# refresh-bio/DSRC

Hardware: AMD Instinct MI355X
Metric: raw FASTQ MB/s compressed (bit-identical .dsrc) at -d3 -q2 (higher is better)
Workload: dtype u8/u16/u32 integer

## Files before the change

### dsrc_amd/csrc/dsrc_gpu.hip

```cpp
#include <hip/hip_runtime.h>

#include <algorithm>
#include <atomic>
#include <cstdarg>
#include <cstdio>
#include <cstdlib>
#include <cstring>
#include <chrono>
#include <condition_variable>
#include <deque>
#include <functional>
#include <dlfcn.h>
#include <mutex>
#ifndef DSRC_REPLAY_WHATIF
#define DSRC_REPLAY_WHATIF 0
#endif
#include <string>
#include <thread>
#include <vector>

#include "../../include/dsrc_gpu.h"
#include "dsrc_types.h"
#include "k_common.h"
#ifndef RCS_WIDE
// ... 656 lines not shown
			hb = std::min(hb, j.key_bits);
			if (j.key_bits > BK_MAX_LB) hb = std::max(hb, j.key_bits - BK_MAX_LB);
			j.bk_hb = hb; j.bk_lb = j.key_bits - hb;
			j.bk_mul = BK_HASH_MUL; j.bk_kmask = (u32)((1ull << j.key_bits) - 1ull);
			j.bk_limit = bk_limit; j.bk_big = bk_big;
			j.bk_narrow_bins = (u32)std::min<long>(BK_MAX_BINS, hook_int("DSRC_GPU_BUCKET_NARROW_BINS", BK_MAX_BINS));
		}
		bk_zero_words = cur;
		o_bk = A.alloc(((size_t)cur + 2 + 128) * 4 + 64);
		size_t cnt_words = 0;
		for (u32 i = 0; i < NJ; ++i)
			if (jobs[i].bk_on)
			{
				if (cnt_words >= (1ull << 32)) return fail(h, DSRCGPU_E_NOMEM, "batch too large for the bucket count table");
				jobs[i].bk_cnt = (u32)cnt_words;
				cnt_words += (((size_t)jobs[i].n + BK_BIN - 1) >> BK_TB) << jobs[i].bk_hb;
			}
		o_bcnt = A.alloc(cnt_words * 2 + 64);
	}
	for (u32 i = 0; i < NJ; ++i) chains[i].bk_on = use_bk ? jobs[i].bk_on : 0u;
	const size_t o_redo = A.alloc(((size_t)NJ + 2) * 4);
	const size_t o_jobs = A.alloc(sizeof(CtxJob) * std::max(1u, NJ)), o_chains = A.alloc(sizeof(RcChain) * std::max(1u, NJ));
	if (A.failed) return fail(h, DSRCGPU_E_NOMEM, "arena exhausted (phase 3b): batch needs > %zu bytes of HBM scratch", A.top);
	CtxJob* d_jobs = AP<CtxJob>(h, o_jobs); RcChain* d_chains = AP<RcChain>(h, o_chains);

	HIPCHK(hipMemcpyAsync(st.data(), d_state, sizeof(BlkState) * B, hipMemcpyDeviceToHost, s));
	HIPCHK(hipStreamSynchronize(s));
	mark("S3"); tr.stage("dsrc batch: tags, order models, range coder");
	std::vector<TagFieldRes> tres((size_t)B * DSRC_MAX_FIELDS);
	memset(tres.data(), 0, sizeof(TagFieldRes) * tres.size());
	size_t tz_lo = al(A.top, 256); A.top = tz_lo;
	for (u32 b = 0; b < B; ++b)
	{
		const BlkState& S = st[b]; BlkDesc& D = desc[b];
		size_t words = 0, hdr = 64;
		tplan[b].rbits_off = (u32)words; words += S.n_recs + 4;
		tplan[b].raw_hist_off = (u32)words; words += 128 + h_huff_ws_words(128) + h_huff_tree_cap(128) / 4 + 16;
		for (u32 fi = 0; fi < S.n_fields && !S.mixed; ++fi)
		{
			const TagField& f = S.fld[fi];
			TagFieldRes& R = tres[(size_t)b * DSRC_MAX_FIELDS + fi];
			hdr += 32 + f.len0 + f.len0 / 8;
			if (f.is_string)
			{
				R.hist_off = (u32)words; words += 129 * 256;
				R.ham_off = (u32)words; words += f.len0 + 4;
				R.code_off = (u32)words; words += 129 * 256;
				R.len_off = (u32)words; words += 129 * 256;
				R.tree_slot = 4 + h_huff_tree_cap(256);
				R.tree_off = (u32)(words * 4); words += ((size_t)129 * R.tree_slot + 3) / 4;
				R.ws_slot = h_huff_ws_words(256); R.ws_off = (u32)words; words += (size_t)129 * R.ws_slot;
				hdr += (size_t)129 * R.tree_slot;
			}
			else if (f.is_numeric && !f.is_constant && f.var_stat_encode)
			{
				R.hist_off = (u32)words; words += 512;
				R.code_off = (u32)words; words += 512;
				R.len_off = (u32)words; words += 512;
				R.tree_slot = 4 + h_huff_tree_cap(512);
				R.tree_off = (u32)(words * 4); words += (R.tree_slot + 3) / 4;
				R.ws_slot = h_huff_ws_words(512); R.ws_off = (u32)words; words += R.ws_slot;
				hdr += R.tree_slot;
			}
		}
		if (S.mixed) hdr += 64 + h_huff_tree_cap(128);
		tplan[b].scr = A.alloc(words * 4) / 4;
		const size_t cap_bytes = hdr + ((size_t)S.raw_tag * 9 + 7) / 8 + (size_t)S.n_recs * ((size_t)S.n_fields * 5 + 8) + 64;
		D.tag_cap = (u32)(al(cap_bytes, 16) / 4 + 4);
		D.tag_out = A.alloc((size_t)D.tag_cap * 4) / 4;
	}
	size_t tz_hi = al(A.top, 256); A.top = tz_hi;
	if (A.failed) return fail(h, DSRCGPU_E_NOMEM, "arena exhausted (tags): batch needs > %zu bytes of HBM scratch", A.top);
	HIPCHK(hipMemsetAsync(h->arena.base + tz_lo, 0, tz_hi - tz_lo, s));
	HIPCHK(hipMemcpyAsync(d_desc, desc.data(), sizeof(BlkDesc) * B, hipMemcpyHostToDevice, s));
	HIPCHK(hipMemcpyAsync(d_tplan, tplan.data(), sizeof(TagPlan) * B, hipMemcpyHostToDevice, s));
	HIPCHK(hipMemcpyAsync(d_tres, tres.data(), sizeof(TagFieldRes) * tres.size(), hipMemcpyHostToDevice, s));
	hipLaunchKernelGGL(k_tag_hist, dim3(B), dim3(WG), 0, s, d_in, d_desc, d_state, rp, wpool, wpool, d_tplan, d_tres); KCHK();
	hipLaunchKernelGGL(k_tag_trees, dim3((DSRC_MAX_FIELDS * DSRC_MAX_STRF + 63) / 64, B), dim3(64), 0, s, d_state, wpool, d_tplan, d_tres); KCHK();
	hipLaunchKernelGGL(k_tag_emit, dim3(B), dim3(WG), 0, s, d_in, d_desc, d_state, rp, wpool, spool, wpool, wpool, d_tplan, d_tres); KCHK();
	hipLaunchKernelGGL(k_tag_raw, dim3(B), dim3(WG), 0, s, d_in, d_desc, d_state, rp, wpool, wpool, d_tplan); KCHK();

	if (zero_hi > zero_lo) HIPCHK(hipMemsetAsync(h->arena.base + zero_lo, 0, zero_hi - zero_lo, s));
	HIPCHK(hipMemcpyAsync(d_desc, desc.data(), sizeof(BlkDesc) * B, hipMemcpyHostToDevice, s));
	HIPCHK(hipMemcpyAsync(d_qplan, qplan.data(), sizeof(QuaPlan) * B, hipMemcpyHostToDevice, s));
	HIPCHK(hipMemcpyAsync(d_dplan, dplan.data(), sizeof(QuaPlan) * B, hipMemcpyHostToDevice, s));
	if (NJ)
	{
		HIPCHK(hipMemcpyAsync(d_jobs, jobs.data(), sizeof(CtxJob) * NJ, hipMemcpyHostToDevice, s));
		HIPCHK(hipMemcpyAsync(d_chains, chains.data(), sizeof(RcChain) * NJ, hipMemcpyHostToDevice, s));
	}

	u32 maxq = 1, maxd = 1, max_len = 1, max_qn = 1;
	for (u32 b = 0; b < B; ++b) { maxq = std::max(maxq, st[b].q_total); maxd = std::max(maxd, st[b].d_total); max_len = std::max(max_len, st[b].max_len); max_qn = std::max(max_qn, st[b].q_count); }

	if (qo == 0)
	{
		hipLaunchKernelGGL(k_qpos_hist, dim3(B), dim3(WG), 0, s, d_desc, d_state, rp, d_q, wpool, d_qplan); KCHK();
		hipLaunchKernelGGL(k_qpos_trees, dim3((max_len + 63) / 64, B), dim3(64), 0, s, d_state, wpool, d_qplan); KCHK();
		hipLaunchKernelGGL(k_qpos_emit, dim3(B), dim3(WG), 0, s, d_desc, d_state, rp, d_q, wpool, wpool, d_qplan); KCHK();
		hipLaunchKernelGGL(k_qrle_runs, dim3(B), dim3(WG), 0, s, d_desc, d_state, d_q, wpool, d_qplan); KCHK();
		hipLaunchKernelGGL(k_qrle_hist, dim3(B), dim3(WG), 0, s, d_desc, d_state, d_q, wpool, d_qplan); KCHK();
		hipLaunchKernelGGL(k_qrle_trees, dim3((2 * max_qn + 63) / 64, B), dim3(64), 0, s, d_state, wpool, d_qplan); KCHK();
		hipLaunchKernelGGL(k_qrle_emit, dim3(B), dim3(WG), 0, s, d_desc, d_state, d_q, wpool, wpool, d_qplan); KCHK();
	}
	if (dna_order == 0)
	{
		const u32 gx = std::max(1u, std::min(64u, (maxd / 4 + WG - 1) / WG));
		hipLaunchKernelGGL(k_dna_b2, dim3(gx, B), dim3(WG), 0, s, d_desc, d_state, d_d, wpool); KCHK();
		hipLaunchKernelGGL(k_dna_huff, dim3(B), dim3(WG), 0, s, d_desc, d_state, d_d, wpool, wpool, d_dplan); KCHK();
	}
	hipLaunchKernelGGL(k_dna_none, dim3((B + 63) / 64), dim3(64), 0, s, d_desc, d_state, wpool, B); KCHK();
	h->rc_launches = 0;
	std::function<int(const BkGroup&)> launch_fallback;
	u32* d_bk = use_bk ? AP<u32>(h, o_bk) : nullptr;
	u32* d_redo = AP<u32>(h, o_redo);
	const bool rc_one_lane = hook_env("DSRC_GPU_RC_ONE_LANE") != nullptr;
	if (NJ)
	{
		const u32 nq = (u32)qjobs.size(), nd = (u32)djobs.size();
		const bool sort_atomic = h->sort_atomic;
		hipLaunchKernelGGL(k_rc_headers, dim3((NJ + 63) / 64), dim3(64), 0, s, d_jobs, NJ, d_state, wpool); KCHK();
		HIPCHK(hipMemsetAsync(d_redo, 0, ((size_t)NJ + 2) * 4, s));
		u16* d_bcnt = use_bk ? AP<u16>(h, o_bcnt) : nullptr;
		if (use_bk) HIPCHK(hipMemsetAsync(d_bk, 0, bk_zero_words * 4, s));
		const u32 max_parts = 2048u;
		launch_fallback = [&, sort_atomic, max_parts](const BkGroup& g) -> int
		{
			const u32 cnt = g.hi - g.lo;
			const u32* fb = d_bk + g.fb;
			if (sort_atomic) hipLaunchKernelGGL((k_sort<0, true>), dim3(std::min(cnt, 16u)), dim3(SORT_WG), 0, s, d_jobs, lpool, d_d, d_q, d_qp, d_state, fb);
			else hipLaunchKernelGGL((k_sort<0, false>), dim3(std::min(cnt, 16u)), dim3(SORT_WG), 0, s, d_jobs, lpool, d_d, d_q, d_qp, d_state, fb);
			u32 mxn = 1; for (u32 i = g.lo; i < g.hi; ++i) mxn = std::max(mxn, jobs[i].n);
			const u32 parts = std::max(1u, std::min(max_parts, mxn / 1024u));
			const dim3 rgrid(parts * std::min(cnt, 4u));
#define BK_REPLAY(NN) { hipLaunchKernelGGL(k_replay_seams<NN>, rgrid, dim3(REPLAY_WG), 0, s, d_jobs, const_cast<u64*>(lpool), parts, cnt, fb); \
					hipLaunchKernelGGL((k_replay<NN, 0>), rgrid, dim3(REPLAY_WG), 0, s, d_jobs, lpool, AP<RcPack>(h, 0), parts, cnt, fb); }
			switch (jobs[g.lo].n_alpha)
			{
			case 4: BK_REPLAY(4) break; case 8: BK_REPLAY(8) break; case 16: BK_REPLAY(16) break;
			case 32: BK_REPLAY(32) break; case 64: BK_REPLAY(64) break; default: BK_REPLAY(128) break;
			}
#undef BK_REPLAY
			KCHK();
			return 0;
		};
		for (size_t sl = 0; sl + 1 < slice_lo.size(); ++sl)
		{
			const u32 s_lo = slice_lo[sl], s_hi = slice_lo[sl + 1];
			stage_mark(0);
			if (use_bk)
			{
				u32 slice_bins = 0;
				for (u32 i = s_lo; i < s_hi; ++i) if (jobs[i].bk_on) slice_bins = std::max(slice_bins, (jobs[i].n + BK_BIN - 1) >> BK_TB);
				hipLaunchKernelGGL(k_part, dim3(std::max(1u, slice_bins), s_hi - s_lo), dim3(PART_WG), 0, s, d_jobs + s_lo, lpool, d_d, d_q, d_qp, d_state, d_bk, d_bcnt);
				KCHK();
				stage_mark(0); stage_mark(1);
				if (slice_bins) { hipLaunchKernelGGL(k_binoff, dim3(slice_bins, s_hi - s_lo), dim3(256), 0, s, d_jobs + s_lo, d_bcnt, d_bk); KCHK(); }
				for (const BkGroup& g : bk_groups[sl])
				{
					u32 hb = 0; bool any = false;
					for (u32 i = g.lo; i < g.hi; ++i) if (jobs[i].bk_on) { any = true; hb = std::max(hb, jobs[i].bk_hb); }
					if (!any) continue;
					u32 lbm = 0; for (u32 i = g.lo; i < g.hi; ++i) if (jobs[i].bk_on) lbm = std::max(lbm, jobs[i].bk_lb);
#define BK_LAUNCH(NN, MB, RB) hipLaunchKernelGGL((k_model<NN, MB, RB>), dim3(((1u << hb) + MD_WAVES_FOR(RB) - 1) / MD_WAVES_FOR(RB), g.hi - g.lo), dim3(64 * MD_WAVES_FOR(RB)), 0, s, d_jobs + g.lo, lpool, AP<RcPack>(h, 0), d_bk, d_bcnt, (RcPack*)(d_bk + ((bk_zero_words + 1) & ~(size_t)1)))
#define BK_FINISH(NN) { if ((1u << lbm) * 4 * MdRow<NN>::STRIDE <= 4096) BK_LAUNCH(NN, 0, 4096); \
						else if ((1u << lbm) * 4 * MdRow<NN>::STRIDE <= MD_ROW_BYTES) BK_LAUNCH(NN, 0, MD_ROW_BYTES); \
						else if (lbm <= 10) BK_LAUNCH(NN, 10, MD_ROW_BYTES); \
						else BK_LAUNCH(NN, BK_MAX_LB, MD_ROW_BYTES); }
					switch (jobs[g.lo].n_alpha)
					{
					case 4: BK_FINISH(4) break; case 8: BK_FINISH(8) break; case 16: BK_FINISH(16) break;
					case 32: BK_FINISH(32) break; case 64: BK_FINISH(64) break; default: BK_FINISH(128) break;
					}
#undef BK_LAUNCH
#undef BK_FINISH
					KCHK();
				}
				if (bk_binned && slice_bins) { hipLaunchKernelGGL(k_place, dim3(slice_bins, s_hi - s_lo), dim3(PLACE_WG), 0, s, d_jobs + s_lo, lpool, AP<RcPack>(h, 0), d_bk); KCHK(); }
				for (const BkGroup& g : bk_groups[sl])
				{
					bool known = false;
					for (u32 i = g.lo; i < g.hi; ++i) known = known || !jobs[i].bk_on;
					if (known) { const int rc = launch_fallback(g); if (rc) return rc; }
				}
				stage_mark(1);
				continue;
			}
#ifdef DSRC_SORT_PROBE
			{
				static int shots = 0;
				if (sl == 0 && shots < 2)
				{
					++shots;
					hipEvent_t e0, e1; hipEventCreate(&e0); hipEventCreate(&e1);
#define PROBE_RUN(M) { hipEventRecord(e0, s); if (sort_atomic) hipLaunchKernelGGL((k_sort<M, true>), dim3(s_hi - s_lo), dim3(SORT_WG), 0, s, d_jobs + s_lo, lpool, d_d, d_q, d_qp, d_state, nullptr); else hipLaunchKernelGGL((k_sort<M, false>), dim3(s_hi - s_lo), dim3(SORT_WG), 0, s, d_jobs + s_lo, lpool, d_d, d_q, d_qp, d_state, nullptr); \
					hipEventRecord(e1, s); hipEventSynchronize(e1); float ms = 0; hipEventElapsedTime(&ms, e0, e1); fprintf(stderr, "[probe] k_sort<%u> %u streams: %.2f ms\n", (unsigned)M, s_hi - s_lo, ms); }
					PROBE_RUN(0) PROBE_RUN(0) PROBE_RUN(128) PROBE_RUN(129) PROBE_RUN(130) PROBE_RUN(132) PROBE_RUN(134) PROBE_RUN(136) PROBE_RUN(144) PROBE_RUN(160) PROBE_RUN(192) PROBE_RUN(255)
					hipEventDestroy(e0); hipEventDestroy(e1);
				}
			}
#endif
			if (sort_atomic) hipLaunchKernelGGL((k_sort<0, true>), dim3(s_hi - s_lo), dim3(SORT_WG), 0, s, d_jobs + s_lo, lpool, d_d, d_q, d_qp, d_state, nullptr);
			else hipLaunchKernelGGL((k_sort<0, false>), dim3(s_hi - s_lo), dim3(SORT_WG), 0, s, d_jobs + s_lo, lpool, d_d, d_q, d_qp, d_state, nullptr);
			KCHK();
			stage_mark(0); stage_mark(1);
			for (u32 lo = s_lo; lo < s_hi;)
			{
				u32 hi = lo;
				while (hi < s_hi && jobs[hi].n_alpha == jobs[lo].n_alpha) ++hi;
				const u32 cnt = hi - lo;
				u32 mxn = 1; for (u32 i = lo; i < hi; ++i) mxn = std::max(mxn, jobs[i].n);
				const u32 parts = std::max(1u, std::min(max_parts, mxn / 1024u));
				const dim3 rgrid(parts * cnt);
#ifdef DSRC_SORT_PROBE
				{
					static int shots = 0;
					if ((jobs[lo].n_alpha == 32 || jobs[lo].n_alpha == 4) && lo == s_lo && shots < 4 && (sl == 0 || sl + 2 == slice_lo.size()))
					{
						++shots;
						hipEvent_t e0, e1; hipEventCreate(&e0); hipEventCreate(&e1);
#define RPROBE_RUN(NN, M) { hipEventRecord(e0, s); hipLaunchKernelGGL((k_replay<NN, M>), rgrid, dim3(REPLAY_WG), 0, s, d_jobs + lo, lpool, AP<RcPack>(h, 0), parts, cnt, nullptr); \
						hipEventRecord(e1, s); hipEventSynchronize(e1); float ms = 0; hipEventElapsedTime(&ms, e0, e1); fprintf(stderr, "[probe] k_replay<%d,%d> %u streams x %u parts: %.2f ms\n", NN, M, cnt, parts, ms); }
						hipLaunchKernelGGL(k_replay_seams<32>, rgrid, dim3(REPLAY_WG), 0, s, d_jobs + lo, const_cast<u64*>(lpool), parts, cnt, nullptr);
						if (jobs[lo].n_alpha == 32) { RPROBE_RUN(32, 0) RPROBE_RUN(32, 0) RPROBE_RUN(32, 1) RPROBE_RUN(32, 2) RPROBE_RUN(32, 8) RPROBE_RUN(32, 16) }
						else { RPROBE_RUN(4, 0) RPROBE_RUN(4, 0) RPROBE_RUN(4, 1) RPROBE_RUN(4, 2) RPROBE_RUN(4, 8) RPROBE_RUN(4, 16) }
						hipEventDestroy(e0); hipEventDestroy(e1);
					}
				}
#endif
				switch (jobs[lo].n_alpha)
				{
				case 4:   hipLaunchKernelGGL(k_replay_seams<4>, rgrid, dim3(REPLAY_WG), 0, s, d_jobs + lo, const_cast<u64*>(lpool), parts, cnt, nullptr); hipLaunchKernelGGL((k_replay<4, DSRC_REPLAY_WHATIF>), rgrid, dim3(REPLAY_WG), 0, s, d_jobs + lo, lpool, AP<RcPack>(h, 0), parts, cnt, nullptr); break;
				case 8:   hipLaunchKernelGGL(k_replay_seams<8>, rgrid, dim3(REPLAY_WG), 0, s, d_jobs + lo, const_cast<u64*>(lpool), parts, cnt, nullptr); hipLaunchKernelGGL((k_replay<8, DSRC_REPLAY_WHATIF>), rgrid, dim3(REPLAY_WG), 0, s, d_jobs + lo, lpool, AP<RcPack>(h, 0), parts, cnt, nullptr); break;
				case 16:  hipLaunchKernelGGL(k_replay_seams<16>, rgrid, dim3(REPLAY_WG), 0, s, d_jobs + lo, const_cast<u64*>(lpool), parts, cnt, nullptr); hipLaunchKernelGGL((k_replay<16, DSRC_REPLAY_WHATIF>), rgrid, dim3(REPLAY_WG), 0, s, d_jobs + lo, lpool, AP<RcPack>(h, 0), parts, cnt, nullptr); break;
				case 32:  hipLaunchKernelGGL(k_replay_seams<32>, rgrid, dim3(REPLAY_WG), 0, s, d_jobs + lo, const_cast<u64*>(lpool), parts, cnt, nullptr); hipLaunchKernelGGL((k_replay<32, DSRC_REPLAY_WHATIF>), rgrid, dim3(REPLAY_WG), 0, s, d_jobs + lo, lpool, AP<RcPack>(h, 0), parts, cnt, nullptr); break;
				case 64:  hipLaunchKernelGGL(k_replay_seams<64>, rgrid, dim3(REPLAY_WG), 0, s, d_jobs + lo, const_cast<u64*>(lpool), parts, cnt, nullptr); hipLaunchKernelGGL((k_replay<64, DSRC_REPLAY_WHATIF>), rgrid, dim3(REPLAY_WG), 0, s, d_jobs + lo, lpool, AP<RcPack>(h, 0), parts, cnt, nullptr); break;
				default:  hipLaunchKernelGGL(k_replay_seams<128>, rgrid, dim3(REPLAY_WG), 0, s, d_jobs + lo, const_cast<u64*>(lpool), parts, cnt, nullptr); hipLaunchKernelGGL((k_replay<128, DSRC_REPLAY_WHATIF>), rgrid, dim3(REPLAY_WG), 0, s, d_jobs + lo, lpool, AP<RcPack>(h, 0), parts, cnt, nullptr); break;
				}
				KCHK();
				lo = hi;
			}
			stage_mark(1);
		}
		HIPCHK(hipEventRecord(h->ev[4], s));
		HIPCHK(hipStreamWaitEvent(h->rc_stream, h->ev[4], 0));
		HIPCHK(hipEventRecord(h->ev[2], h->rc_stream));
		if (rc_one_lane) hipLaunchKernelGGL(k_rc, dim3((NJ + RC_LANES - 1) / RC_LANES), dim3(64 * RC_WG_WAVES), 0, h->rc_stream, d_chains, NJ, (const u32*)nullptr, AP<RcPack>(h, 0), wpool, d_state);
		else if (NJ > (u32)hook_int("DSRC_GPU_RC_WIDE_FROM", 640)) hipLaunchKernelGGL(k_rcs<RCS_WIDE>, dim3((NJ + RCS_WIDE - 1) / RCS_WIDE), dim3(64 * RCS_WG_WAVES), 0, h->rc_stream, d_chains, NJ, AP<RcPack>(h, 0), wpool, d_state, (const u32*)d_bk, d_redo);
		else hipLaunchKernelGGL(k_rcs<16>, dim3((NJ + 15) / 16), dim3(64 * RCS_WG_WAVES), 0, h->rc_stream, d_chains, NJ, AP<RcPack>(h, 0), wpool, d_state, (const u32*)d_bk, d_redo);
		KCHK();
		HIPCHK(hipEventRecord(h->ev[3], h->rc_stream));
		HIPCHK(hipEventSynchronize(h->ev[3]));
		h->rc_launches = 1;
	}

	hipLaunchKernelGGL(k_meta_plan, dim3((B + 63) / 64), dim3(64), 0, s, d_state, prm); KCHK();

	HIPCHK(hipMemcpyAsync(st.data(), d_state, sizeof(BlkState) * B, hipMemcpyDeviceToHost, s));
	std::vector<u32> bk_flags, redo;
	if (NJ)
	{
		redo.resize((size_t)NJ + 1); HIPCHK(hipMemcpyAsync(redo.data(), d_redo, ((size_t)NJ + 1) * 4, hipMemcpyDeviceToHost, s));
		if (use_bk) { bk_flags.resize(NJ); HIPCHK(hipMemcpyAsync(bk_flags.data(), d_bk, (size_t)NJ * 4, hipMemcpyDeviceToHost, s)); }
	}
	HIPCHK(hipStreamSynchronize(s));
	if (NJ && !rc_one_lane)
	{
		std::vector<u32> list(redo.begin() + 1, redo.begin() + 1 + std::min<u32>(redo[0], NJ));
		u32 why[4] = {0, 0, 0, 0};
		for (u32& x : list) { ++why[(x >> 28) & 3u]; x &= 0x0FFFFFFFu; }
		bool handed = false;
		for (u32 i = 0; i < NJ && use_bk; ++i) if (bk_flags[i] && jobs[i].bk_on) { list.push_back(i); handed = true; }
		if (!list.empty())
		{
			mark("redo"); tr.stage("dsrc batch: range coder, redo list");
			if (handed)
				for (size_t sl = 0; sl + 1 < slice_lo.size(); ++sl)
					for (const BkGroup& g : bk_groups[sl])
					{
						bool any = false;
						for (u32 i = g.lo; i < g.hi; ++i) any = any || (bk_flags[i] && jobs[i].bk_on);
						if (any) { const int rc = launch_fallback(g); if (rc) return rc; }
					}
			std::sort(list.begin(), list.end()); list.erase(std::unique(list.begin(), list.end()), list.end());
			std::vector<u32> up(list.size() + 1); up[0] = (u32)list.size(); std::copy(list.begin(), list.end(), up.begin() + 1);
			HIPCHK(hipMemcpyAsync(d_redo, up.data(), up.size() * 4, hipMemcpyHostToDevice, s));
			hipLaunchKernelGGL(k_rc, dim3(((u32)list.size() + RC_LANES - 1) / RC_LANES), dim3(64 * RC_WG_WAVES), 0, s, d_chains, NJ, (const u32*)d_redo, AP<RcPack>(h, 0), wpool, d_state); KCHK();
			HIPCHK(hipMemcpyAsync(st.data(), d_state, sizeof(BlkState) * B, hipMemcpyDeviceToHost, s));
			HIPCHK(hipStreamSynchronize(s));
			h->rc_redone += (u32)list.size();
			if (getenv("DSRC_GPU_DEBUG")) fprintf(stderr, "[dsrc_gpu] range coder: %zu of %u streams coded again by k_rc (%u carry clamps: fix row taken %u, recovery refused %u, forced %u; the others handed back by the bucketed front end)\n", list.size(), NJ, std::min<u32>(redo[0], NJ), why[1], why[2], why[3]);
		}
	}
	mark("S4"); tr.stage("dsrc batch: assemble");
	if (!bk_flags.empty() && getenv("DSRC_GPU_DEBUG"))
	{
		u32 on = 0, back = 0;
		for (u32 i = 0; i < NJ; ++i) { on += jobs[i].bk_on; back += bk_flags[i] && jobs[i].bk_on; }
		fprintf(stderr, "[dsrc_gpu] bucketed path: %u of %u streams tried, %u handed back to k_sort / k_replay\n", on, NJ, back);
	}
	u64 total = 0;
	for (u32 b = 0; b < B; ++b)
	{
		const BlkState& S = st[b];
		if ((S.err & DSRC_ERR_OUT_OVERFLOW) && !h->rc_caps_worst && NJ)
		{
			h->rc_caps_worst = true; A.failed = true;
			return fail(h, DSRCGPU_E_NOMEM, "chunk %u: a range-coded stream outgrew its staging estimate; the batch is run again with worst-case staging", b);
// ... 1375 lines not shown
```

### dsrc_amd/csrc/k_bucket.h

```cpp
#pragma once
#include <type_traits>
#include "k_rc.h"

#define BK_MAX_HB 10
#define BK_MAX_LB 11
#define BK_LIMIT 524288
#define BK_BIG 16384
#ifndef BK_TB
#define BK_TB 13
#endif
#define BK_BIN (1u << BK_TB)
static_assert(BK_TB == RC6_TB, "a time bin is the unit of k_rc's record layout (rc6_chunk_off)");
#ifndef BK_MAX_BINS
#define BK_MAX_BINS 512
#endif
#define BK_MAX_BINS_WIDE 65536
#define BK_HASH_MUL 0x9E3779B1u


__device__ __forceinline__ u64 bk_rekey(const CtxJob& j, u64 el)
{
	const u32 key = ((u32)(el >> ELEM_CTX_SHIFT) * j.bk_mul) & j.bk_kmask;
	return (el & ((1ull << ELEM_CTX_SHIFT) - 1ull)) | ((u64)key << ELEM_CTX_SHIFT);
}

__device__ __forceinline__ void bk_fallback(const CtxJob& j, u32* bk)
{
	if (atomicExch(&bk[j.jid], 1u) != 0u) return;
	const u32 k = atomicAdd(&bk[j.bk_fb], 1u);
	bk[j.bk_fb + 1 + k] = j.jid;
}

__device__ __forceinline__ bool bk_fast8(const CtxJob& j) { return j.is_dna ? (j.alpha_bits == 2 && j.order <= 9) : j.order <= 4; }

struct BkWin { u64 a, b, c; };
__device__ __forceinline__ BkWin bk_load8(const CtxJob& j, const u8* s, u32 t0)
{
	BkWin w;
	if (j.is_dna) { w.a = *(const u64_unaligned*)(s + t0 - 9); w.b = *(const u64_unaligned*)(s + t0 - 1); w.c = *(const u64_unaligned*)(s + t0); }
	else { w.a = *(const u64_unaligned*)(s + t0 - 8); w.b = 0; w.c = *(const u64_unaligned*)(s + t0); }
	return w;
}

__device__ __forceinline__ void bk_elems8_dna(const CtxJob& j, const BkWin& w, u32 t0, u64* el, bool* bad)
{
	const u64 wa = w.a, wb = w.b, wc = w.c;
	if ((wa | wc) & 0xFCFCFCFCFCFCFCFCull) *bad = true;
	const u32 P = (pack2x8(__builtin_bswap64(wa)) << 16) | pack2x8(__builtin_bswap64(wb));
	const u32 cmask = (u32)((1ull << (2 * j.order)) - 1ull);
#pragma unroll
	for (u32 i = 0; i < 8; ++i)
	{
		const u32 ctx = (P >> (14 - 2 * i)) & cmask;
		const u32 key = (ctx * j.bk_mul) & j.bk_kmask;
		el[i] = ((u64)key << ELEM_CTX_SHIFT) | ((u64)((u32)(wc >> (8 * i)) & 3u) << ELEM_SYM_SHIFT) | (t0 + i);
	}
}

__device__ __forceinline__ void bk_elems8_qua(const CtxJob& j, const BkWin& w, const u8* qp, const u8* rank, u32 t0, u64* el)
{
	const u32 ab = j.alpha_bits, order = j.order, half = order / 2;
	const u64 w0 = w.a, w1 = w.c;
	u32 r[16];
#pragma unroll
	for (u32 m = 0; m < 8; ++m) { r[m] = rank[(u32)(w0 >> (8 * m)) & 0xFFu]; r[8 + m] = rank[(u32)(w1 >> (8 * m)) & 0xFFu]; }
	u32 pos = j.qlen ? t0 - exact_div(t0, j.qm_lo, j.qm_hi) * j.qlen : 0u;
#pragma unroll
	for (u32 i = 0; i < 8; ++i)
	{
		u32 h = 0;
#pragma unroll
		for (u32 k = 4; k >= 1; --k)
			if (k <= order)
			{
				const u32 slot = k - 1;
				const u32 x = (slot < half || order == 1) ? r[7 + i - slot] : ((r[7 + i - slot] + r[6 + i - slot]) >> 1);
				h = (h << ab) | x;
			}
		const u32 pctx = (j.qlen ? exact_div(pos * 128u, j.qm_lo, j.qm_hi) : (u32)qp[t0 + i]) >> j.rescale_shift;
		const u32 key = ((((h << ab) | pctx)) * j.bk_mul) & j.bk_kmask;
		el[i] = ((u64)key << ELEM_CTX_SHIFT) | ((u64)(r[8 + i] & ((1u << ab) - 1u)) << ELEM_SYM_SHIFT) | (t0 + i);
		pos = pos + 1 == j.qlen ? 0u : pos + 1;
	}
}

#ifndef PART_ITEMS
#define PART_ITEMS 16
#endif
#define PART_WG (BK_BIN / PART_ITEMS)
#ifndef PART_PASSES
#define PART_PASSES 1
#endif
#define PART_WAVES (PART_WG / 64)
#define BK_EL_SYM_SHIFT BK_TB
#define BK_EL_KEY_SHIFT (BK_TB + 7)
static_assert(BK_EL_KEY_SHIFT + BK_MAX_LB <= 32, "low key bits, symbol and time inside the tile in 32 bits");
__device__ __forceinline__ u32 bk_keysym(u64 e) { return ((u32)(e >> (ELEM_SYM_SHIFT + 1)) & ~0x7Fu) | ((u32)(e >> ELEM_SYM_SHIFT) & 0x7Fu); }
static_assert(ELEM_CTX_SHIFT == ELEM_SYM_SHIFT + 8, "bk_keysym");

__global__ void __launch_bounds__(PART_WG) k_part(const CtxJob* jobs, u64* pool, const u8* d_stream, const u8* q_stream, const u8* qp_stream, BlkState* st, u32* bk, u16* bcnt)
{
	__shared__ u16 s_cnt[PART_WAVES][SORT_MAX_BINS];
	__shared__ u32 s_tile[BK_BIN / PART_PASSES];
	__shared__ u32 s_ws[PART_WAVES];
	__shared__ u8 s_rank[256];
	constexpr u32 tile_elems = PART_WG * PART_ITEMS;
	const CtxJob j = jobs[blockIdx.y];
	if (!j.bk_on) { if (blockIdx.x == 0 && threadIdx.x == 0) bk_fallback(j, bk); return; }
	const u32 tile = blockIdx.x * tile_elems;
	if (tile >= j.n) return;
	const u32 n = j.n, bins = 1u << j.bk_hb, lb = j.bk_lb;
	const u32 wv = wave_id(), lane = lane_id();
	const u8* sym_src = (j.is_dna ? d_stream : q_stream) + j.src_off;
	const u8* qp = qp_stream + j.src_off;

	for (u32 i = threadIdx.x; i < 256; i += blockDim.x) s_rank[i] = (!j.is_dna && j.translate) ? st[j.blk].q_sym[i] : (u8)i;
	for (u32 i = threadIdx.x; i < PART_WAVES * SORT_MAX_BINS / 2; i += blockDim.x) ((u32*)&s_cnt[0][0])[i] = 0;
	__syncthreads();

	u32 ks[PART_ITEMS], rk[PART_ITEMS];
	const u32 wbase = tile + wv * 64 * PART_ITEMS;
	bool bad = false;
	if (bk_fast8(j) && tile > 0 && tile + tile_elems + 8 <= n)
	{
		static_assert(PART_ITEMS % 8 == 0, "eight consecutive symbols per lane and round");
		static_assert(PART_WAVES * 512 <= BK_BIN / PART_PASSES, "a strip of 512 elements per wave");
		u32* strip = s_tile + wv * 512;
		BkWin w = bk_load8(j, sym_src, wbase + 8 * lane);
#pragma unroll
		for (u32 h = 0; h < PART_ITEMS / 8; ++h)
		{
			u64 e8[8];
			const u32 t0 = wbase + 512 * h + 8 * lane;
			const BkWin wc = w;
			if (h + 1 < PART_ITEMS / 8) w = bk_load8(j, sym_src, t0 + 512);
			if (j.is_dna) bk_elems8_dna(j, wc, t0, e8, &bad); else bk_elems8_qua(j, wc, qp, s_rank, t0, e8);
			if (h) wave_fence();
#pragma unroll
			for (u32 k = 0; k < 8; ++k) strip[8 * lane + k] = bk_keysym(e8[k]);
			wave_fence();
#pragma unroll
			for (u32 k = 0; k < 8; ++k) ks[8 * h + k] = strip[64 * k + lane];
		}
	}
	else
	{
#pragma unroll
		for (u32 k = 0; k < PART_ITEMS; ++k)
		{
			const u32 i = wbase + k * 64 + lane;
			ks[k] = 0;
			if (i < n)
			{
				const u64 e = bk_rekey(j, j.is_dna ? ctx_elem_dna(j, sym_src, i, &bad) : ctx_elem_qua(j, sym_src, qp, s_rank, i));
				ks[k] = bk_keysym(e);
			}
		}
	}
	if (bad) atomicOr(&st[j.blk].err, (u32)DSRC_ERR_REF_UB);
	const u32 shift = 7 + lb;
#pragma unroll
	for (u32 k = 0; k < PART_ITEMS; ++k)
	{
		const u32 i = wbase + k * 64 + lane;
		const u32 d = ks[k] >> shift;
		const u32 sh = (d & 1u) * 16u;
		u32 old = 0;
		if (i < n) old = atomicAdd(&((u32*)s_cnt[wv])[d >> 1], 1u << sh);
		rk[k] = (old >> sh) & 0xFFFFu;
#ifdef DSRC_EMU_BUILD
		(void)__ballot(true);
#endif
	}
	__syncthreads();
	for (u32 d0 = 0, carry = 0; d0 < bins; d0 += PART_WG)
	{
		const u32 dd = d0 + threadIdx.x;
		u32 c[PART_WAVES], tot = 0;
#pragma unroll
		for (u32 w = 0; w < PART_WAVES; ++w) { c[w] = dd < bins ? s_cnt[w][dd] : 0u; tot += c[w]; }
		const u32 inc = wave_incl_scan_dpp(tot);
		if (lane == 63) s_ws[wv] = inc;
		__syncthreads();
		u32 run = carry + inc - tot;
		const u32 nws = (bins - d0 + 63) / 64 < PART_WAVES ? (bins - d0 + 63) / 64 : PART_WAVES;
		for (u32 i = 0; i < nws; ++i) { const u32 x = s_ws[i]; run += i < wv ? x : 0u; carry += x; }
		if (dd < bins)
		{
			bcnt[(u64)j.bk_cnt + (u64)blockIdx.x * bins + dd] = (u16)tot;
#pragma unroll
			for (u32 w = 0; w < PART_WAVES; ++w) { s_cnt[w][dd] = (u16)run; run += c[w]; }
		}
		if (d0 + PART_WG < bins) __syncthreads();
	}
	__syncthreads();
	const u32 lbmask = (1u << lb) - 1u;
	u32* dst = (u32*)(pool + j.elems) + tile;
	const u32 tile_n = n - tile < tile_elems ? n - tile : tile_elems;
	constexpr u32 PIECE = BK_BIN / PART_PASSES;
#pragma unroll
	for (u32 k = 0; k < PART_ITEMS; ++k) rk[k] += (u32)s_cnt[wv][ks[k] >> shift];
#pragma unroll
	for (u32 p = 0; p < PART_PASSES; ++p)
	{
#pragma unroll
		for (u32 k = 0; k < PART_ITEMS; ++k)
		{
			const u32 i = wbase + k * 64 + lane;
			const u32 at = rk[k] - p * PIECE;
			if (i < n && at < PIECE)
				s_tile[at] = (((ks[k] >> 7) & lbmask) << BK_EL_KEY_SHIFT) | ((ks[k] & 0x7Fu) << BK_EL_SYM_SHIFT) | (i & (BK_BIN - 1u));
		}
		__syncthreads();
		if (tile_n == tile_elems)
		{
#pragma unroll
			for (u32 k = 0; k < PIECE / 2 / PART_WG; ++k) ((u64*)(dst + p * PIECE))[k * PART_WG + threadIdx.x] = ((const u64*)s_tile)[k * PART_WG + threadIdx.x];
		}
		else for (u32 q = threadIdx.x; q < PIECE && p * PIECE + q < tile_n; q += PART_WG) dst[p * PIECE + q] = s_tile[q];
		if (p + 1 < PART_PASSES) __syncthreads();
	}
}

#define MD_WAVES_FOR(ROW_BYTES) ((ROW_BYTES) <= 4096 ? 4 : 2)
#define MD_ROW_BYTES 8192
#define MD_NONE 0xFFFFFFFFu

template <int N> struct MdRow
{
	static constexpr int B = N <= 4 ? 2 : N <= 8 ? 3 : N <= 16 ? 4 : N <= 32 ? 5 : N <= 64 ? 6 : 7;
	static constexpr int L4 = B / 2;
	static constexpr bool R2 = (B & 1) != 0;
	static constexpr u32 W64 = ((1u << (2 * L4)) - 1u) / 3u;
	static constexpr u32 STRIDE = 2 * W64 + (R2 ? N / 2 : 0);
};

template <int N> __device__ __forceinline__ u32 md_init_word(u32 x)
{
	typedef MdRow<N> G;
	if (x >= 2 * G::W64) return 0x00010001u;
	const u32 w = x >> 1;
	const u32 l = w >= 5 ? 2u : w >= 1 ? 1u : 0u;
	const u32 v = (u32)N >> (2 * (l + 1));
	return v | (v << 16);
}

template <int N> __device__ __forceinline__ u32 md_total(const u32* row)
{
	const u64 v = *(const unsigned long long*)row;
	return ((u32)v & 0xFFFFu) + ((u32)v >> 16) + ((u32)(v >> 32) & 0xFFFFu) + (u32)(v >> 48);
}

template <int N> __device__ __forceinline__ void md_rescale(u32* row)
{
	typedef MdRow<N> G;
	unsigned long long* r64 = (unsigned long long*)row;
	if (G::R2)
		for (u32 x = 0; x < (u32)N / 2; ++x)
		{
			const u32 v = row[2 * G::W64 + x];
			u32 a = v & 0xFFFFu, b = v >> 16;
			a -= a >> 1; b -= b >> 1;
			row[2 * G::W64 + x] = a | (b << 16);
		}
	for (int l = G::L4 - 1; l >= 0; --l)
	{
		const u32 base = ((1u << (2 * l)) - 1u) / 3u, nw = 1u << (2 * l);
		for (u32 w = 0; w < nw; ++w)
		{
			u64 v = 0;
			if (!G::R2 && l == G::L4 - 1)
			{
				const u64 o = r64[base + w];
#pragma unroll
				for (u32 q = 0; q < 4; ++q) { u32 x = (u32)(o >> (16 * q)) & 0xFFFFu; x -= x >> 1; v |= (u64)x << (16 * q); }
			}
			else
			{
#pragma unroll
				for (u32 q = 0; q < 4; ++q)
				{
					const u32 c = 4 * w + q;
					u32 sum;
					if (l == G::L4 - 1) { const u32 p = row[2 * G::W64 + c]; sum = (p & 0xFFFFu) + (p >> 16); }
					else { const u64 o = r64[((1u << (2 * (l + 1))) - 1u) / 3u + c]; sum = ((u32)o & 0xFFFFu) + ((u32)o >> 16) + ((u32)(o >> 32) & 0xFFFFu) + (u32)(o >> 48); }
					v |= (u64)sum << (16 * q);
				}
			}
			r64[base + w] = v;
		}
	}
}

template <int N> __device__ __forceinline__ u64 md_code(u32* row, u32 sym)
{
	typedef MdRow<N> G;
	unsigned long long* r64 = (unsigned long long*)row;
	u32 cum = 0, tot = 0, f = 0;
#pragma unroll
	for (int l = 0; l < G::L4; ++l)
	{
		const u32 q = (sym >> (G::B - 2 * l - 2)) & 3u;
		const u32 wi = ((1u << (2 * l)) - 1u) / 3u + (l ? sym >> (G::B - 2 * l) : 0u);
		const u64 old = atomicAdd(&r64[wi], 2ull << (16 * q));
		const u64 below = old & ((1ull << (16 * q)) - 1ull);
		cum += ((u32)below & 0xFFFFu) + ((u32)below >> 16) + ((u32)(below >> 32) & 0xFFFFu);
		if (l == 0) tot = ((u32)old & 0xFFFFu) + ((u32)old >> 16) + ((u32)(old >> 32) & 0xFFFFu) + (u32)(old >> 48);
		f = (u32)(old >> (16 * q)) & 0xFFFFu;
	}
	if (G::R2)
	{
		const u32 old = atomicAdd(&row[2 * G::W64 + (sym >> 1)], (sym & 1u) ? (2u << 16) : 2u);
		cum += (sym & 1u) ? (old & 0xFFFFu) : 0u;
		f = (sym & 1u) ? (old >> 16) : (old & 0xFFFFu);
	}
	return (u64)f | ((u64)cum << 16) | ((u64)tot << 32);
}

__global__ void __launch_bounds__(256) k_binoff(const CtxJob* jobs, u16* bcnt, const u32* bk)
{
	const CtxJob j = jobs[blockIdx.y];
	const u32 bin = blockIdx.x;
	if (!j.bk_on || bk[j.jid] || (bin << BK_TB) >= j.n) return;
	const u32 bins = 1u << j.bk_hb;
	u16* row = bcnt + j.bk_cnt + (u64)bin * bins;
	u32 c[4], mine = 0;
#pragma unroll
	for (u32 k = 0; k < 4; ++k)
	{
		const u32 b = 4 * threadIdx.x + k;
		c[k] = b < bins ? (u32)row[b] : 0u;
		mine += c[k];
	}
	u32 tot;
	u32 run = block_excl_scan(mine, &tot);
#pragma unroll
	for (u32 k = 0; k < 4; ++k)
	{
		const u32 b = 4 * threadIdx.x + k;
		if (b < bins) row[b] = (u16)run;
		run += c[k];
	}
}

template <bool SMALL> struct MdMapT { typedef u8 T; static constexpr u32 NONE = 0xFFu, CLAIM = 0x80u; };
template <> struct MdMapT<false> { typedef u16 T; static constexpr u32 NONE = 0xFFFFu, CLAIM = 0x8000u; };

#ifndef MD_AHEAD
#define MD_AHEAD 3
#endif
#ifndef MD_ROTATE_ALL
#define MD_ROTATE_ALL 0
#endif
template <int N, int MAPBITS, int ROW_BYTES>
__global__ void __launch_bounds__(64 * MD_WAVES_FOR(ROW_BYTES)) k_model(const CtxJob* jobs, const u64* pool, RcPack* rec_pool, u32* bk, const u16* bcnt, RcPack* nowhere)
{
	constexpr u32 STRIDE = MdRow<N>::STRIDE;
	constexpr u32 ROWS = ROW_BYTES / (4 * STRIDE);
	constexpr u32 MD_WAVES = MD_WAVES_FOR(ROW_BYTES);
	typedef MdMapT<(ROWS <= 127)> Map;
	typedef typename Map::T map_t;
	__shared__ map_t s_map[MD_WAVES][1 << MAPBITS];
	__shared__ unsigned long long s_rows[MD_WAVES][ROW_BYTES / 8];
	__shared__ u16 s_off[MD_WAVES][BK_MAX_BINS];
	__shared__ u16 s_num[MD_WAVES][BK_MAX_BINS];
	__shared__ u8 s_head[MD_WAVES][64];
	constexpr u32 limit = (1u << 16) - 2u * N;
	const CtxJob j = jobs[blockIdx.y];
	const u32 w = wave_id(), lane = lane_id();
#ifndef MD_XCD_MAP
#define MD_XCD_MAP 1
#endif
	u32 bx = blockIdx.x;
	if (MD_XCD_MAP && gridDim.x % 8u == 0) bx = (((bx & 7u) + blockIdx.y) & 7u) * (gridDim.x >> 3) + (bx >> 3);
// ... 257 lines not shown
```

Measured before the change: 65670.

## Specialize k_part by stream kind and order, tabulate position contexts

Templates the partition kernel on stream kind (two-bit DNA, quality with a fixed order, or generic) and launches one instance per run of jobs with the same kind and order, so the context build runs fully unrolled without per-element branches. Quality position contexts come from a shared-memory table built once per block (or from the stream or a division), replacing a per-element exact division. The key hash uses a 24-bit multiply, and full inner tiles skip bounds checks when ranking and scattering. In exchange there are more kernel launches per slice and a debug getenv call on the host for each one.

```diff
diff --git a/dsrc_amd/csrc/dsrc_gpu.hip b/dsrc_amd/csrc/dsrc_gpu.hip
--- a/dsrc_amd/csrc/dsrc_gpu.hip
+++ b/dsrc_amd/csrc/dsrc_gpu.hip
@@ -832,8 +832,32 @@
 			{
 				u32 slice_bins = 0;
 				for (u32 i = s_lo; i < s_hi; ++i) if (jobs[i].bk_on) slice_bins = std::max(slice_bins, (jobs[i].n + BK_BIN - 1) >> BK_TB);
-				hipLaunchKernelGGL(k_part, dim3(std::max(1u, slice_bins), s_hi - s_lo), dim3(PART_WG), 0, s, d_jobs + s_lo, lpool, d_d, d_q, d_qp, d_state, d_bk, d_bcnt);
-				KCHK();
+				for (const BkGroup& g : bk_groups[sl])
+					for (u32 lo = g.lo, hi; lo < g.hi; lo = hi)
+					{
+						u32 order = 0, o2 = 0;
+						const BkKind kind = bk_kind(jobs[lo], &order);
+						for (hi = lo + 1; hi < g.hi && bk_kind(jobs[hi], &o2) == kind && o2 == order; ++hi);
+						u32 run_bins = 1;
+						for (u32 i = lo; i < hi; ++i) if (jobs[i].bk_on) run_bins = std::max(run_bins, (jobs[i].n + BK_BIN - 1) >> BK_TB);
+#define BK_PART(KIND, ORDER) hipLaunchKernelGGL((k_part<KIND, ORDER>), dim3(run_bins, hi - lo), dim3(PART_WG), 0, s, d_jobs + lo, lpool, d_d, d_q, d_qp, d_state, d_bk, d_bcnt)
+						if (kind == BK_KIND_DNA2) BK_PART(BK_KIND_DNA2, 0);
+						else if (kind == BK_KIND_ANY) BK_PART(BK_KIND_ANY, 0);
+						else switch (order)
+						{
+						case 1: BK_PART(BK_KIND_QUA, 1); break; case 2: BK_PART(BK_KIND_QUA, 2); break;
+						case 3: BK_PART(BK_KIND_QUA, 3); break; default: BK_PART(BK_KIND_QUA, 4); break;
+						}
+#undef BK_PART
+						KCHK();
+						if (getenv("DSRC_GPU_DEBUG"))
+						{
+							u32 from[3] = {0, 0, 0};
+							for (u32 i = lo; i < hi; ++i) if (jobs[i].bk_on && jobs[i].n >= 2 * BK_BIN + 8) ++from[bk_pctx(jobs[i])];
+							if (kind == BK_KIND_QUA) fprintf(stderr, "[dsrc_gpu] k_part<qualities, order %u>: %u streams; position context of the inner tiles from the table %u, by division %u, from the stream %u\n", order, hi - lo, from[BK_PCTX_TABLE], from[BK_PCTX_DIV], from[BK_PCTX_STREAM]);
+							else fprintf(stderr, "[dsrc_gpu] k_part<%s>: %u streams\n", kind == BK_KIND_DNA2 ? "two-bit DNA" : "any", hi - lo);
+						}
+					}
 				stage_mark(0); stage_mark(1);
 				if (slice_bins) { hipLaunchKernelGGL(k_binoff, dim3(slice_bins, s_hi - s_lo), dim3(256), 0, s, d_jobs + s_lo, d_bcnt, d_bk); KCHK(); }
 				for (const BkGroup& g : bk_groups[sl])
diff --git a/dsrc_amd/csrc/k_bucket.h b/dsrc_amd/csrc/k_bucket.h
--- a/dsrc_amd/csrc/k_bucket.h
+++ b/dsrc_amd/csrc/k_bucket.h
@@ -18,9 +18,12 @@
 #define BK_HASH_MUL 0x9E3779B1u
 
 
+static_assert(BK_MAX_HB + BK_MAX_LB <= 21, "bk_key: the key lies inside the low 24 bits of the product");
+__device__ __forceinline__ u32 bk_key(u32 ctx, u32 mul, u32 kmask) { return ((ctx & 0xFFFFFFu) * (mul & 0xFFFFFFu)) & kmask; }
+
 __device__ __forceinline__ u64 bk_rekey(const CtxJob& j, u64 el)
 {
-	const u32 key = ((u32)(el >> ELEM_CTX_SHIFT) * j.bk_mul) & j.bk_kmask;
+	const u32 key = bk_key((u32)(el >> ELEM_CTX_SHIFT), j.bk_mul, j.bk_kmask);
 	return (el & ((1ull << ELEM_CTX_SHIFT) - 1ull)) | ((u64)key << ELEM_CTX_SHIFT);
 }
 
@@ -31,18 +34,32 @@
 	bk[j.bk_fb + 1 + k] = j.jid;
 }
 
-__device__ __forceinline__ bool bk_fast8(const CtxJob& j) { return j.is_dna ? (j.alpha_bits == 2 && j.order <= 9) : j.order <= 4; }
+enum BkKind { BK_KIND_ANY = 0, BK_KIND_DNA2 = 1, BK_KIND_QUA = 2 };
+__host__ __device__ inline BkKind bk_kind(const CtxJob& j, u32* order)
+{
+	*order = 0;
+	if (j.is_dna) return (j.alpha_bits == 2 && j.order <= 9) ? BK_KIND_DNA2 : BK_KIND_ANY;
+	if (j.order < 1 || j.order > 4) return BK_KIND_ANY;
+	*order = j.order;
+	return BK_KIND_QUA;
+}
+
+#define PCTX_CAP 1024
+enum BkPctx { BK_PCTX_TABLE = 0, BK_PCTX_DIV = 1, BK_PCTX_STREAM = 2 };
+__host__ __device__ inline BkPctx bk_pctx(const CtxJob& j) { return j.qlen == 0 ? BK_PCTX_STREAM : j.qlen <= PCTX_CAP ? BK_PCTX_TABLE : BK_PCTX_DIV; }
+__device__ __forceinline__ u32 bk_pctx_of(const CtxJob& j, u32 pos) { return exact_div(pos * 128u, j.qm_lo, j.qm_hi) >> j.rescale_shift; }
+
 
 struct BkWin { u64 a, b, c; };
-__device__ __forceinline__ BkWin bk_load8(const CtxJob& j, const u8* s, u32 t0)
+template <bool DNA> __device__ __forceinline__ BkWin bk_load8(const u8* s, u32 t0)
 {
 	BkWin w;
-	if (j.is_dna) { w.a = *(const u64_unaligned*)(s + t0 - 9); w.b = *(const u64_unaligned*)(s + t0 - 1); w.c = *(const u64_unaligned*)(s + t0); }
+	if (DNA) { w.a = *(const u64_unaligned*)(s + t0 - 9); w.b = *(const u64_unaligned*)(s + t0 - 1); w.c = *(const u64_unaligned*)(s + t0); }
 	else { w.a = *(const u64_unaligned*)(s + t0 - 8); w.b = 0; w.c = *(const u64_unaligned*)(s + t0); }
 	return w;
 }
 
-__device__ __forceinline__ void bk_elems8_dna(const CtxJob& j, const BkWin& w, u32 t0, u64* el, bool* bad)
+__device__ __forceinline__ void bk_elems8_dna(const CtxJob& j, const BkWin& w, u32* ks, bool* bad)
 {
 	const u64 wa = w.a, wb = w.b, wc = w.c;
 	if ((wa | wc) & 0xFCFCFCFCFCFCFCFCull) *bad = true;
@@ -52,35 +69,41 @@
 	for (u32 i = 0; i < 8; ++i)
 	{
 		const u32 ctx = (P >> (14 - 2 * i)) & cmask;
-		const u32 key = (ctx * j.bk_mul) & j.bk_kmask;
-		el[i] = ((u64)key << ELEM_CTX_SHIFT) | ((u64)((u32)(wc >> (8 * i)) & 3u) << ELEM_SYM_SHIFT) | (t0 + i);
-	}
-}
-
-__device__ __forceinline__ void bk_elems8_qua(const CtxJob& j, const BkWin& w, const u8* qp, const u8* rank, u32 t0, u64* el)
-{
-	const u32 ab = j.alpha_bits, order = j.order, half = order / 2;
+		ks[i] = (bk_key(ctx, j.bk_mul, j.bk_kmask) << 7) | ((u32)(wc >> (8 * i)) & 3u);
+	}
+}
+
+template <int ORDER, int PCTX>
+__device__ __forceinline__ void bk_elems8_qua(const CtxJob& j, const BkWin& w, const u8* qp, const u8* rank, const u8* pctx_tab, u32 t0, u32* ks)
+{
+	static_assert(ORDER >= 1 && ORDER <= 4, "the ranks of s[t0-8 ..] reach back far enough for four slots");
+	constexpr u32 order = ORDER, half = order / 2;
+	const u32 ab = j.alpha_bits;
 	const u64 w0 = w.a, w1 = w.c;
 	u32 r[16];
 #pragma unroll
 	for (u32 m = 0; m < 8; ++m) { r[m] = rank[(u32)(w0 >> (8 * m)) & 0xFFu]; r[8 + m] = rank[(u32)(w1 >> (8 * m)) & 0xFFu]; }
-	u32 pos = j.qlen ? t0 - exact_div(t0, j.qm_lo, j.qm_hi) * j.qlen : 0u;
+	u32 pos = 0;
+	u64 q8 = 0;
+	if (PCTX == BK_PCTX_STREAM) q8 = *(const u64_unaligned*)(qp + t0);
+	else pos = t0 - exact_div(t0, j.qm_lo, j.qm_hi) * j.qlen;
 #pragma unroll
 	for (u32 i = 0; i < 8; ++i)
 	{
 		u32 h = 0;
 #pragma unroll
-		for (u32 k = 4; k >= 1; --k)
-			if (k <= order)
-			{
-				const u32 slot = k - 1;
-				const u32 x = (slot < half || order == 1) ? r[7 + i - slot] : ((r[7 + i - slot] + r[6 + i - slot]) >> 1);
-				h = (h << ab) | x;
-			}
-		const u32 pctx = (j.qlen ? exact_div(pos * 128u, j.qm_lo, j.qm_hi) : (u32)qp[t0 + i]) >> j.rescale_shift;
-		const u32 key = ((((h << ab) | pctx)) * j.bk_mul) & j.bk_kmask;
-		el[i] = ((u64)key << ELEM_CTX_SHIFT) | ((u64)(r[8 + i] & ((1u << ab) - 1u)) << ELEM_SYM_SHIFT) | (t0 + i);
-		pos = pos + 1 == j.qlen ? 0u : pos + 1;
+		for (u32 k = order; k >= 1; --k)
+		{
+			const u32 slot = k - 1;
+			const u32 x = (slot < half || order == 1) ? r[7 + i - slot] : ((r[7 + i - slot] + r[6 + i - slot]) >> 1);
+			h = (h << ab) | x;
+		}
+		u32 pctx;
+		if (PCTX == BK_PCTX_TABLE) pctx = pctx_tab[pos];
+		else if (PCTX == BK_PCTX_DIV) pctx = bk_pctx_of(j, pos);
+		else pctx = ((u32)(q8 >> (8 * i)) & 0xFFu) >> j.rescale_shift;
+		ks[i] = (bk_key((h << ab) | pctx, j.bk_mul, j.bk_kmask) << 7) | (r[8 + i] & ((1u << ab) - 1u) & 0x7Fu);
+		if (PCTX != BK_PCTX_STREAM) pos = pos + 1 == j.qlen ? 0u : pos + 1;
 	}
 }
 
@@ -97,13 +120,16 @@
 static_assert(BK_EL_KEY_SHIFT + BK_MAX_LB <= 32, "low key bits, symbol and time inside the tile in 32 bits");
 __device__ __forceinline__ u32 bk_keysym(u64 e) { return ((u32)(e >> (ELEM_SYM_SHIFT + 1)) & ~0x7Fu) | ((u32)(e >> ELEM_SYM_SHIFT) & 0x7Fu); }
 static_assert(ELEM_CTX_SHIFT == ELEM_SYM_SHIFT + 8, "bk_keysym");
-
+static_assert(BK_EL_KEY_SHIFT == BK_EL_SYM_SHIFT + 7, "the element is mixed key << 7 | symbol, shifted");
+
+template <int KIND, int ORDER>
 __global__ void __launch_bounds__(PART_WG) k_part(const CtxJob* jobs, u64* pool, const u8* d_stream, const u8* q_stream, const u8* qp_stream, BlkState* st, u32* bk, u16* bcnt)
 {
 	__shared__ u16 s_cnt[PART_WAVES][SORT_MAX_BINS];
 	__shared__ u32 s_tile[BK_BIN / PART_PASSES];
 	__shared__ u32 s_ws[PART_WAVES];
 	__shared__ u8 s_rank[256];
+	__shared__ u8 s_pctx[KIND == BK_KIND_QUA ? PCTX_CAP : 4];
 	constexpr u32 tile_elems = PART_WG * PART_ITEMS;
 	const CtxJob j = jobs[blockIdx.y];
 	if (!j.bk_on) { if (blockIdx.x == 0 && threadIdx.x == 0) bk_fallback(j, bk); return; }
@@ -111,37 +137,50 @@
 	if (tile >= j.n) return;
 	const u32 n = j.n, bins = 1u << j.bk_hb, lb = j.bk_lb;
 	const u32 wv = wave_id(), lane = lane_id();
-	const u8* sym_src = (j.is_dna ? d_stream : q_stream) + j.src_off;
+	const bool is_dna = KIND == BK_KIND_ANY ? j.is_dna != 0 : KIND == BK_KIND_DNA2;
+	const u8* sym_src = (is_dna ? d_stream : q_stream) + j.src_off;
 	const u8* qp = qp_stream + j.src_off;
-
-	for (u32 i = threadIdx.x; i < 256; i += blockDim.x) s_rank[i] = (!j.is_dna && j.translate) ? st[j.blk].q_sym[i] : (u8)i;
+	const bool inner = KIND != BK_KIND_ANY && tile > 0 && tile + tile_elems + 8 <= n;
+	const BkPctx pctx_from = bk_pctx(j);
+
+	for (u32 i = threadIdx.x; i < 256; i += blockDim.x) s_rank[i] = (!is_dna && j.translate) ? st[j.blk].q_sym[i] : (u8)i;
 	for (u32 i = threadIdx.x; i < PART_WAVES * SORT_MAX_BINS / 2; i += blockDim.x) ((u32*)&s_cnt[0][0])[i] = 0;
+	if (KIND == BK_KIND_QUA && inner && pctx_from == BK_PCTX_TABLE)
+		for (u32 pos = threadIdx.x; pos < j.qlen; pos += blockDim.x) s_pctx[pos] = (u8)bk_pctx_of(j, pos);
 	__syncthreads();
 
 	u32 ks[PART_ITEMS], rk[PART_ITEMS];
 	const u32 wbase = tile + wv * 64 * PART_ITEMS;
 	bool bad = false;
-	if (bk_fast8(j) && tile > 0 && tile + tile_elems + 8 <= n)
+	if (inner)
 	{
 		static_assert(PART_ITEMS % 8 == 0, "eight consecutive symbols per lane and round");
 		static_assert(PART_WAVES * 512 <= BK_BIN / PART_PASSES, "a strip of 512 elements per wave");
 		u32* strip = s_tile + wv * 512;
-		BkWin w = bk_load8(j, sym_src, wbase + 8 * lane);
-#pragma unroll
-		for (u32 h = 0; h < PART_ITEMS / 8; ++h)
-		{
-			u64 e8[8];
-			const u32 t0 = wbase + 512 * h + 8 * lane;
-			const BkWin wc = w;
-			if (h + 1 < PART_ITEMS / 8) w = bk_load8(j, sym_src, t0 + 512);
-			if (j.is_dna) bk_elems8_dna(j, wc, t0, e8, &bad); else bk_elems8_qua(j, wc, qp, s_rank, t0, e8);
-			if (h) wave_fence();
-#pragma unroll
-			for (u32 k = 0; k < 8; ++k) strip[8 * lane + k] = bk_keysym(e8[k]);
-			wave_fence();
-#pragma unroll
-			for (u32 k = 0; k < 8; ++k) ks[8 * h + k] = strip[64 * k + lane];
-		}
+		auto make = [&](auto pctx_tag)
+		{
+			constexpr int PCTX = decltype(pctx_tag)::value;
+			BkWin w = bk_load8<KIND == BK_KIND_DNA2>(sym_src, wbase + 8 * lane);
+#pragma unroll
+			for (u32 h = 0; h < PART_ITEMS / 8; ++h)
+			{
+				u32 e8[8];
+				const u32 t0 = wbase + 512 * h + 8 * lane;
+				const BkWin wc = w;
+				if (h + 1 < PART_ITEMS / 8) w = bk_load8<KIND == BK_KIND_DNA2>(sym_src, t0 + 512);
+				if constexpr (KIND == BK_KIND_DNA2) bk_elems8_dna(j, wc, e8, &bad);
+				else if constexpr (KIND == BK_KIND_QUA) bk_elems8_qua<ORDER, PCTX>(j, wc, qp, s_rank, s_pctx, t0, e8);
+				if (h) wave_fence();
+#pragma unroll
+				for (u32 k = 0; k < 8; ++k) strip[8 * lane + k] = e8[k];
+				wave_fence();
+#pragma unroll
+				for (u32 k = 0; k < 8; ++k) ks[8 * h + k] = strip[64 * k + lane];
+			}
+		};
+		if (KIND != BK_KIND_QUA || pctx_from == BK_PCTX_TABLE) make(std::integral_constant<int, BK_PCTX_TABLE>());
+		else if (pctx_from == BK_PCTX_DIV) make(std::integral_constant<int, BK_PCTX_DIV>());
+		else make(std::integral_constant<int, BK_PCTX_STREAM>());
 	}
 	else
 	{
@@ -152,74 +191,79 @@
 			ks[k] = 0;
 			if (i < n)
 			{
-				const u64 e = bk_rekey(j, j.is_dna ? ctx_elem_dna(j, sym_src, i, &bad) : ctx_elem_qua(j, sym_src, qp, s_rank, i));
+				const u64 e = bk_rekey(j, is_dna ? ctx_elem_dna(j, sym_src, i, &bad) : ctx_elem_qua(j, sym_src, qp, s_rank, i));
 				ks[k] = bk_keysym(e);
 			}
 		}
 	}
 	if (bad) atomicOr(&st[j.blk].err, (u32)DSRC_ERR_REF_UB);
-	const u32 shift = 7 + lb;
-#pragma unroll
-	for (u32 k = 0; k < PART_ITEMS; ++k)
-	{
-		const u32 i = wbase + k * 64 + lane;
-		const u32 d = ks[k] >> shift;
-		const u32 sh = (d & 1u) * 16u;
-		u32 old = 0;
-		if (i < n) old = atomicAdd(&((u32*)s_cnt[wv])[d >> 1], 1u << sh);
-		rk[k] = (old >> sh) & 0xFFFFu;
+	auto finish = [&](auto full_tag)
+	{
+		constexpr bool FULL = decltype(full_tag)::value;
+		const u32 shift = 7 + lb;
+#pragma unroll
+		for (u32 k = 0; k < PART_ITEMS; ++k)
+		{
+			const u32 i = wbase + k * 64 + lane;
+			const u32 pair = (ks[k] >> (shift + 1));
+			const u32 sh = (ks[k] >> (shift - 4)) & 16u;
+			u32 old = 0;
+			if (FULL || i < n) old = atomicAdd(&((u32*)s_cnt[wv])[pair], 1u << sh);
+			rk[k] = (old >> sh) & 0xFFFFu;
 #ifdef DSRC_EMU_BUILD
-		(void)__ballot(true);
-#endif
-	}
-	__syncthreads();
-	for (u32 d0 = 0, carry = 0; d0 < bins; d0 += PART_WG)
-	{
-		const u32 dd = d0 + threadIdx.x;
-		u32 c[PART_WAVES], tot = 0;
-#pragma unroll
-		for (u32 w = 0; w < PART_WAVES; ++w) { c[w] = dd < bins ? s_cnt[w][dd] : 0u; tot += c[w]; }
-		const u32 inc = wave_incl_scan_dpp(tot);
-		if (lane == 63) s_ws[wv] = inc;
+			(void)__ballot(true);
+#endif
+		}
 		__syncthreads();
-		u32 run = carry + inc - tot;
-		const u32 nws = (bins - d0 + 63) / 64 < PART_WAVES ? (bins - d0 + 63) / 64 : PART_WAVES;
-		for (u32 i = 0; i < nws; ++i) { const u32 x = s_ws[i]; run += i < wv ? x : 0u; carry += x; }
-		if (dd < bins)
-		{
-			bcnt[(u64)j.bk_cnt + (u64)blockIdx.x * bins + dd] = (u16)tot;
-#pragma unroll
-			for (u32 w = 0; w < PART_WAVES; ++w) { s_cnt[w][dd] = (u16)run; run += c[w]; }
-		}
-		if (d0 + PART_WG < bins) __syncthreads();
-	}
-	__syncthreads();
-	const u32 lbmask = (1u << lb) - 1u;
-	u32* dst = (u32*)(pool + j.elems) + tile;
-	const u32 tile_n = n - tile < tile_elems ? n - tile : tile_elems;
-	constexpr u32 PIECE = BK_BIN / PART_PASSES;
-#pragma unroll
-	for (u32 k = 0; k < PART_ITEMS; ++k) rk[k] += (u32)s_cnt[wv][ks[k] >> shift];
-#pragma unroll
-	for (u32 p = 0; p < PART_PASSES; ++p)
-	{
-#pragma unroll
-		for (u32 k = 0; k < PART_ITEMS; ++k)
-		{
-			const u32 i = wbase + k * 64 + lane;
-			const u32 at = rk[k] - p * PIECE;
-			if (i < n && at < PIECE)
-				s_tile[at] = (((ks[k] >> 7) & lbmask) << BK_EL_KEY_SHIFT) | ((ks[k] & 0x7Fu) << BK_EL_SYM_SHIFT) | (i & (BK_BIN - 1u));
+		for (u32 d0 = 0, carry = 0; d0 < bins; d0 += PART_WG)
+		{
+			const u32 dd = d0 + threadIdx.x;
+			u32 c[PART_WAVES], tot = 0;
+#pragma unroll
+			for (u32 w = 0; w < PART_WAVES; ++w) { c[w] = dd < bins ? s_cnt[w][dd] : 0u; tot += c[w]; }
+			const u32 inc = wave_incl_scan_dpp(tot);
+			if (lane == 63) s_ws[wv] = inc;
+			__syncthreads();
+			u32 run = carry + inc - tot;
+			const u32 nws = (bins - d0 + 63) / 64 < PART_WAVES ? (bins - d0 + 63) / 64 : PART_WAVES;
+			for (u32 i = 0; i < nws; ++i) { const u32 x = s_ws[i]; run += i < wv ? x : 0u; carry += x; }
+			if (dd < bins)
+			{
+				bcnt[(u64)j.bk_cnt + (u64)blockIdx.x * bins + dd] = (u16)tot;
+#pragma unroll
+				for (u32 w = 0; w < PART_WAVES; ++w) { s_cnt[w][dd] = (u16)run; run += c[w]; }
+			}
+			if (d0 + PART_WG < bins) __syncthreads();
 		}
 		__syncthreads();
-		if (tile_n == tile_elems)
-		{
-#pragma unroll
-			for (u32 k = 0; k < PIECE / 2 / PART_WG; ++k) ((u64*)(dst + p * PIECE))[k * PART_WG + threadIdx.x] = ((const u64*)s_tile)[k * PART_WG + threadIdx.x];
-		}
-		else for (u32 q = threadIdx.x; q < PIECE && p * PIECE + q < tile_n; q += PART_WG) dst[p * PIECE + q] = s_tile[q];
-		if (p + 1 < PART_PASSES) __syncthreads();
-	}
+		const u32 elmask = (((1u << lb) - 1u) << 7) | 0x7Fu;
+		u32* dst = (u32*)(pool + j.elems) + tile;
+		const u32 tile_n = n - tile < tile_elems ? n - tile : tile_elems;
+		constexpr u32 PIECE = BK_BIN / PART_PASSES;
+#pragma unroll
+		for (u32 k = 0; k < PART_ITEMS; ++k) rk[k] += (u32)s_cnt[wv][ks[k] >> shift];
+#pragma unroll
+		for (u32 p = 0; p < PART_PASSES; ++p)
+		{
+#pragma unroll
+			for (u32 k = 0; k < PART_ITEMS; ++k)
+			{
+				const u32 i = wbase + k * 64 + lane;
+				const u32 at = rk[k] - p * PIECE;
+				if ((FULL && PART_PASSES == 1) || (i < n && at < PIECE))
+					s_tile[at] = ((ks[k] & elmask) << BK_EL_SYM_SHIFT) | (wv * 64 * PART_ITEMS + k * 64 + lane);
+			}
+			__syncthreads();
+			if (FULL || tile_n == tile_elems)
+			{
+#pragma unroll
+				for (u32 k = 0; k < PIECE / 2 / PART_WG; ++k) ((u64*)(dst + p * PIECE))[k * PART_WG + threadIdx.x] = ((const u64*)s_tile)[k * PART_WG + threadIdx.x];
+			}
+			else for (u32 q = threadIdx.x; q < PIECE && p * PIECE + q < tile_n; q += PART_WG) dst[p * PIECE + q] = s_tile[q];
+			if (p + 1 < PART_PASSES) __syncthreads();
+		}
+	};
+	if (inner) finish(std::true_type()); else finish(std::false_type());
 }
 
 #define MD_WAVES_FOR(ROW_BYTES) ((ROW_BYTES) <= 4096 ? 4 : 2)
```

After: 67570, median of 6. +2.9%, better.
